# Ocheretovich/tachyon

Measured on AMD Instinct MI355X. Metric: BN254 G1 MSM scalars/s @2^26 and Fr NTT elems/s @2^24, 1/2/4/8 GPU, higher is better.
Workload: dtype u32; 1 GPU; BN254 G1 VariableBaseMSM 2^26 (BASELINE configs[1]), device-resident inputs, result normalised to affine on the host; msm_log_n=26, points_per_gpu=67108864, window_bits=21, windows=12, windows_per_gpu=12, parallelism=msm point shards x1 + RCCL all-gather of partial points, communicator=single GPU

## Files before the change

### include/tachyon_mi355x.h

```cpp
#ifndef TACHYON_MI355X_H_
#define TACHYON_MI355X_H_

#include <stddef.h>
#include <stdint.h>

#define TACHYON_C_EXPORT __attribute__((visibility("default")))

#ifdef __cplusplus
extern "C" {
#endif

typedef struct tachyon_bn254_fq { uint64_t limbs[4]; } tachyon_bn254_fq;
typedef struct tachyon_bn254_fr { uint64_t limbs[4]; } tachyon_bn254_fr;
typedef struct tachyon_bn254_fq2 { tachyon_bn254_fq c0, c1; } tachyon_bn254_fq2;
typedef struct tachyon_bls12_381_fq { uint64_t limbs[6]; } tachyon_bls12_381_fq;
typedef struct tachyon_bls12_381_fr { uint64_t limbs[4]; } tachyon_bls12_381_fr;
typedef struct tachyon_bls12_381_fq2 { tachyon_bls12_381_fq c0, c1; } tachyon_bls12_381_fq2;

#define TACHYON_MI355X_POINT_TYPES(C, G, F)                                   \
  typedef struct tachyon_##C##_##G##_affine { F x, y; } tachyon_##C##_##G##_affine;             \
  typedef struct tachyon_##C##_##G##_point2 { F x, y; } tachyon_##C##_##G##_point2;             \
  typedef struct tachyon_##C##_##G##_jacobian { F x, y, z; } tachyon_##C##_##G##_jacobian;      \
  typedef struct tachyon_##C##_##G##_projective { F x, y, z; } tachyon_##C##_##G##_projective;  \
  typedef struct tachyon_##C##_##G##_xyzz { F x, y, zz, zzz; } tachyon_##C##_##G##_xyzz;
// ... 398 lines not shown
typedef struct tachyon_mi355x_msm_shard {
  size_t start, count;
  unsigned point_groups, window_groups, window_bits, w_begin, w_end;
} tachyon_mi355x_msm_shard;
TACHYON_C_EXPORT int tachyon_mi355x_msm_shard_plan(int curve, size_t n_total, int world, int rank,
                                                  tachyon_mi355x_msm_shard* out);
TACHYON_C_EXPORT int tachyon_mi355x_msm_gpu_sharded_plan_affine(int curve, void* ctx, tachyon_mi355x_comm* comm,
                                                                const tachyon_mi355x_msm_shard* plan,
                                                                const void* bases, const void* scalars,
                                                                void* out_affine);
TACHYON_C_EXPORT int tachyon_mi355x_msm_gpu_run_points(int curve, void* ctx, const void* bases, size_t bases_size,
                                                      int base_form, const void* scalars, size_t scalars_size,
                                                      int form, void* out);
TACHYON_C_EXPORT void tachyon_mi355x_msm_gpu_set_window_bits(int curve, void* ctx, unsigned c);
TACHYON_C_EXPORT int tachyon_mi355x_msm_gpu_set_mixed_windows(int curve, void* ctx, unsigned windows);
TACHYON_C_EXPORT int tachyon_mi355x_msm_mixed_layout(int curve, unsigned windows, unsigned* c_lo, unsigned* n_wide,
                                                     unsigned* key_bits, unsigned* bit_offsets,
                                                     unsigned* bucket_offsets);
TACHYON_C_EXPORT void tachyon_mi355x_msm_gpu_set_profile(int curve, void* ctx, int on);
TACHYON_C_EXPORT int tachyon_mi355x_msm_gpu_set_variant(int curve, void* ctx, int variant);
TACHYON_C_EXPORT void tachyon_mi355x_msm_gpu_last_timings(int curve, const void* ctx, float* out8);
TACHYON_C_EXPORT size_t tachyon_mi355x_msm_gpu_last_divisions(int curve, const void* ctx);
TACHYON_C_EXPORT size_t tachyon_mi355x_msm_gpu_run_bytes(int curve, const void* ctx, size_t size, size_t batch_count);
TACHYON_C_EXPORT size_t tachyon_mi355x_msm_gpu_held_bytes(int curve, const void* ctx);
TACHYON_C_EXPORT unsigned tachyon_mi355x_msm_gpu_last_schedule(int curve, const void* ctx);
TACHYON_C_EXPORT double tachyon_mi355x_msm_madd_ceiling(int curve, int field_bits);
TACHYON_C_EXPORT int tachyon_mi355x_msm_gpu_set_devices(int curve, void* ctx, const int* device_ids, size_t count);
TACHYON_C_EXPORT size_t tachyon_mi355x_msm_gpu_last_shards(int curve, const void* ctx, float* shard_ms,
                                                           size_t* shard_points, int* shard_devices, size_t cap);
TACHYON_C_EXPORT void tachyon_mi355x_msm_plan(int curve, size_t size, unsigned* c, unsigned* windows);
// ... 215 lines not shown
```

### tachyon_amd/_lib.py

```python
import ctypes
import os

HERE = os.path.dirname(os.path.abspath(__file__))
LIB_PATH = os.environ.get("TACHYON_MI355X_LIB") or os.path.join(HERE, "libtachyon_mi355x.so")

CURVES = {"bn254_g1": 0, "bn254_g2": 1, "bls12_381_g1": 2, "bls12_381_g2": 3}
FIELDS = {"bn254_fq": 0, "bn254_fr": 1, "bls12_381_fq": 2, "bls12_381_fr": 3}
FIELD_BYTES = {"bn254_fq": 32, "bn254_fr": 32, "bls12_381_fq": 48, "bls12_381_fr": 32}
CURVE_INFO = {
    "bn254_g1": (64, "bn254_fr"),
    "bn254_g2": (128, "bn254_fr"),
    "bls12_381_g1": (96, "bls12_381_fr"),
    "bls12_381_g2": (192, "bls12_381_fr"),
}

_lib = None

vp, sz, i32, u8, u64 = ctypes.c_void_p, ctypes.c_size_t, ctypes.c_int, ctypes.c_uint8, ctypes.c_uint64
fp = ctypes.POINTER(ctypes.c_float)
COMM_FN = ctypes.CFUNCTYPE(ctypes.c_int, ctypes.c_void_p, ctypes.c_void_p, ctypes.c_void_p, ctypes.c_size_t)


class MsmShard(ctypes.Structure):
    _fields_ = [("start", ctypes.c_size_t), ("count", ctypes.c_size_t), ("point_groups", ctypes.c_uint),
# ... 95 lines not shown
    ("tachyon_mi355x_ntt4_split_log_r", ctypes.c_uint32, [ctypes.c_uint32, ctypes.c_uint32]),
    ("tachyon_mi355x_bn254_ntt4_stage", None, [vp, i32, i32, vp, vp]),
    ("tachyon_mi355x_bn254_ntt4_synchronize", None, [vp]),
    ("tachyon_mi355x_bn254_ntt4_stream", vp, [vp]),
    ("tachyon_bn254_g2_create_msm_gpu", vp, [u8]),
    ("tachyon_bn254_g2_destroy_msm_gpu", None, [vp]),
    ("tachyon_bn254_g2_affine_msm_gpu", vp, [vp, vp, vp, sz]),
    ("tachyon_bls12_381_g2_create_msm_gpu", vp, [u8]),
    ("tachyon_bls12_381_g2_destroy_msm_gpu", None, [vp]),
    ("tachyon_bls12_381_g2_affine_msm_gpu", vp, [vp, vp, vp, sz]),
    ("tachyon_mi355x_msm_gpu_affine", None, [i32, vp, vp, vp, sz, vp]),
    ("tachyon_mi355x_msm_gpu_window_range_affine", None, [i32, vp, vp, vp, sz, ctypes.c_uint, ctypes.c_uint, vp]),
    ("tachyon_mi355x_msm_gpu_batch_affine", i32, [i32, vp, vp, sz, vp, sz, vp]),
    ("tachyon_mi355x_msm_gpu_plan_windows", ctypes.c_uint, [i32, vp, sz]),
    ("tachyon_mi355x_msm_gpu_set_mixed_windows", i32, [i32, vp, ctypes.c_uint]),
    ("tachyon_mi355x_msm_mixed_layout", i32, [i32, ctypes.c_uint] + [vp] * 5),
    ("tachyon_mi355x_msm_gpu_fold_bases", i32, [i32, vp, vp, sz, ctypes.c_uint, vp]),
    ("tachyon_mi355x_msm_gpu_folded_affine", i32, [i32, vp, vp, vp, sz, ctypes.c_uint, vp]),
    ("tachyon_mi355x_msm_gpu_create", vp, [i32, vp]),
    ("tachyon_mi355x_msm_gpu_destroy", None, [i32, vp]),
    ("tachyon_mi355x_msm_gpu_run", i32, [i32, vp, vp, sz, vp, sz, i32, vp]),
    ("tachyon_mi355x_msm_gpu_run_points", i32, [i32, vp, vp, sz, i32, vp, sz, i32, vp]),
    ("tachyon_mi355x_msm_gpu_set_window_bits", None, [i32, vp, ctypes.c_uint]),
    ("tachyon_mi355x_msm_gpu_set_profile", None, [i32, vp, i32]),
    ("tachyon_mi355x_msm_gpu_set_variant", i32, [i32, vp, i32]),
    ("tachyon_mi355x_msm_gpu_last_divisions", sz, [i32, vp]),
    ("tachyon_mi355x_msm_gpu_run_bytes", sz, [i32, vp, sz, sz]),
    ("tachyon_mi355x_msm_gpu_held_bytes", sz, [i32, vp]),
    ("tachyon_mi355x_msm_gpu_last_schedule", ctypes.c_uint, [i32, vp]),
    ("tachyon_mi355x_msm_madd_ceiling", ctypes.c_double, [i32, i32]),
# ... 194 lines not shown
```

### tachyon_amd/csrc/capi/capi_msm.hip

```cpp
#include "../../../include/tachyon_mi355x.h"

#include <algorithm>
#include <cstdio>
#include <cstdlib>
#include <cstring>
#include <memory>
#include <string>
#include <vector>

#include "../dist/comm.h"
#include "../msm/msm.h"
#include "../msm/msm_multi.h"
#include "capi_guard.h"

using namespace tachyon_amd;

namespace {

template <class Curve>
struct MsmCtx {
  msm::MsmGpu<Curve> impl;
  std::unique_ptr<msm::MsmMultiDevice<Curve>> multi;
  std::string input_dir;
  bool log = false;
// ... 494 lines not shown
}
int tachyon_mi355x_msm_gpu_set_mixed_windows(int curve, void* ctx, unsigned windows) {
  if (!ctx || curve < 0 || curve > 3) return 0;
  const unsigned bits = curve < 2 ? Bn254Fr::Config::kModulusBits : Bls381Fr::Config::kModulusBits;
  if (windows && !msm::MsmPlan::mixed_layout_ok(bits, windows)) return 0;
  GUARD_BEGIN
  CURVE_DISPATCH(curve, {
    auto* m = static_cast<MsmCtx<C>*>(ctx);
    if (windows && m->impl.force_window_bits()) return 0;
    if (windows && window_groups_set(m->impl.variant())) return 0;
    m->set([&](auto& g) { g.set_mixed_windows(windows); });
  })
  GUARD_END
  return 1;
}
int tachyon_mi355x_msm_mixed_layout(int curve, unsigned windows, unsigned* c_lo, unsigned* n_wide, unsigned* key_bits,
                                    unsigned* bit_offsets, unsigned* bucket_offsets) {
  if (curve < 0 || curve > 3) return 0;
  const unsigned bits = curve < 2 ? Bn254Fr::Config::kModulusBits : Bls381Fr::Config::kModulusBits;
  if (!msm::MsmPlan::mixed_layout_ok(bits, windows)) return 0;
  GUARD_BEGIN
  const msm::MsmPlan p = msm::MsmPlan::make_mixed(1, bits, windows);
  if (c_lo) *c_lo = p.c;
  if (n_wide) *n_wide = p.n_wide;
  if (key_bits) *key_bits = msm::kMixedKeyBits;
  for (unsigned w = 0; w <= windows; ++w) {
    if (bit_offsets) bit_offsets[w] = p.bit_offset(w);
    if (bucket_offsets) bucket_offsets[w] = (unsigned)p.bucket_offset(w);
  }
  GUARD_END
// ... 109 lines not shown
```

### tachyon_amd/csrc/msm/msm.h

```cpp
#pragma once
#include <hip/hip_runtime.h>

#include <cstddef>
#include <algorithm>
#include <cstdint>
#include <cstdlib>
#include <stdexcept>
#include <string>
#include <vector>

#include "../common/hip_util.h"
#include "../ec/point.h"

namespace tachyon_amd::msm {

constexpr int kMsmVariantMask = 0x3FFFFBF | (1 << 27);
constexpr int kMsmVariantUniformWindows = 1 << 27;
constexpr unsigned kSchedFusedRecode = 1, kSchedRecodeFedSort = 2, kSchedNarrowStaging = 4, kSchedAcc29 = 8,
                   kSchedLanePair = 16, kSchedAcc28 = 32, kSchedChainsChecked = 64, kSchedEntStaged = 128,
                   kSchedMixedWindows = 256;

constexpr unsigned kMixedKeyBits = 24;
constexpr uint32_t kMixedNoKey = (1u << kMixedKeyBits) - 1;

// ... 172 lines not shown
  static size_t fold_table_bytes(size_t points, unsigned fold) { return (size_t)fold * points * sizeof(Aff); }
  static size_t fold_staging_bytes(size_t points, unsigned fold);
  static constexpr size_t kFoldChunkBytes = size_t(1) << 30;

  static Point combine_windows(const std::vector<Point>& window_sums, unsigned c);
  static Point combine_windows(const std::vector<Point>& window_sums, const MsmPlan& plan);
  static double madd_ceiling(int field_bits);

  void set_force_window_bits(unsigned c) { force_c_ = c; }
  void set_mixed_windows(unsigned W) {
    if (W && !MsmPlan::mixed_layout_ok(Fr::Config::kModulusBits, W))
      (void)MsmPlan::make_mixed(1, Fr::Config::kModulusBits, W);
    mixed_w_ = W;
  }
  unsigned mixed_windows() const { return mixed_w_; }
  void set_variant(int v) {
    if (v < 0 || (v & ~kMsmVariantMask)) throw std::runtime_error("tachyon_mi355x: unknown MSM variant bits");
    variant_ = v;
  }
  void set_profile(bool on) { profile_ = on; }
  unsigned force_window_bits() const { return force_c_; }
  int variant() const { return variant_; }
  bool profile() const { return profile_; }
  const MsmTimings& timings() const { return timings_; }
  hipStream_t stream() const { return stream_; }
  unsigned last_levels() const { return last_levels_; }
  size_t last_divisions() const { return last_divisions_; }
  unsigned last_schedule() const { return last_schedule_; }

 private:
// ... 10 lines not shown
  Buffers carve(const Shape& s);
  uint32_t* recode(const Shape& s, const Buffers& b, const Fr* d_scalars);
  void sort_group(const Shape& s, const Buffers& b, unsigned g, size_t e0, size_t ecount, uint32_t* digit_off);
  void upload_pending_bases(const Aff* d_bases, size_t n);
  void early_chain_tables(const Shape& s, const Buffers& b, size_t e0, size_t ecount);
  AccLaunch acc_launch(bool raw, int ent_mode) const;
  void accumulate(const Shape& s, const Buffers& b, const Aff* d_bases, unsigned g, size_t e0, size_t ecount,
                  size_t tbase);
  ReduceKernels reduce_kernels(bool raw) const;
  void check_early_flags(const Shape& s, const Buffers& b);
  void join_offsets(const Shape& s, const Buffers& b, uint32_t nchains, unsigned K2, unsigned levels, uint32_t* ltab,
                    size_t stride);
  void join(const Shape& s, const Buffers& b, const ReduceKernels& rk);
  void window_sums_two_level(const Shape& s, const Buffers& b, const ReduceKernels& rk, Point* d_windows);
  void window_sums_by_trees(const Shape& s, const Buffers& b, Point* d_windows);
  void window_sums(const Shape& s, const Buffers& b, const ReduceKernels& rk, Point* d_windows);
  void window_sums_by_segments(const Shape& s, const Buffers& b, const ReduceKernels& rk, Point* d_windows);
  Point run_host_pipelined(const void* bases, const void* scalars, size_t n, size_t chunks);
  size_t work_bytes(size_t n, unsigned c, size_t batch = 1) const;
  MsmPlan run_plan(size_t n, unsigned c) const;
  struct AccFields {
    bool tree_reduce, acc29, acc28, pair_acc, pair_limb;
  };
  static AccFields acc_fields(int variant);
  struct SlotBytes {
    size_t slot, lvl_slot;
    bool raw;
  };
  static SlotBytes slot_bytes(const AccFields& f, int variant);
  static bool window_sums_by_scan(const AccFields& f, unsigned buckets);
  static unsigned class_seg(unsigned windows, unsigned buckets);
  static size_t mixed_seg_sums(const AccFields& f, unsigned narrow, unsigned W, unsigned B);
  struct SortKnobs {
    bool fuse_recode, rocprim_hist, wide_stage;
    uint32_t spt;
  };
  static SortKnobs sort_knobs(int variant);
  struct SortShape {
    unsigned key_bits, sort_begin, places;
    uint32_t spt;
    bool narrow, fused, own_sort;
    size_t scatter_lds;
  };
  static SortShape sort_shape(const SortKnobs& k, unsigned c, unsigned Ws, unsigned W, unsigned G, size_t entries,
                              bool mixed = false);
  size_t memory_divisions(size_t n, size_t resident_bytes) const;
  void ensure_group_events(unsigned groups);
  void build_chains(const Shape& s, const Buffers& b);
  hipError_t sort_entries(void* tmp, size_t& bytes, const uint64_t* in, uint64_t* out, size_t count,
                          unsigned begin_bit, unsigned end_bit, hipStream_t s);

  hipStream_t stream_ = nullptr;
  bool own_stream_ = false;
  bool profile_ = false;
  unsigned force_c_ = 0;
  unsigned mixed_w_ = 0;
  int variant_ = 0;
  MsmTimings timings_;
  DeviceBuffer bases_, scalars_, ents_, ents2_, sort_tmp_, scan_tmp_, check_;
  DeviceBuffer start_, end_, cnt_, off_a_, off_b_, part_a_, part_b_, seg_a_, seg_b_, windows_, buckets_;
  enum Mark {
    kMarkStart,
    kMarkUploaded,
    kMarkRecoded,
    kMarkSorted,
    kMarkAccumulated,
    kMarkEnd,
    kMarkChainsRead,
    kMarks
  };
  hipEvent_t ev_[kMarks] = {};
// ... 32 lines not shown
```

### tachyon_amd/csrc/msm/msm_impl.h

```cpp
#pragma once
#include "msm.h"
#include "../field/f29.h"
#include "acc29.h"
#include "acc28.h"
#include "acc_pair.h"
#include "pair28.h"
#include "pair29.h"

#include <rocprim/device/device_radix_sort.hpp>
#include <rocprim/device/device_scan.hpp>

#include <algorithm>
#include <cmath>
#include <condition_variable>
#include <cstdlib>
#include <exception>
#include <mutex>
#include <thread>

namespace tachyon_amd::msm {

namespace detail {
namespace {

// ... 436 lines not shown
      k.rsum_pass1 = &window_rsum_pair_kernel<Curve, Fips>;
      k.rsum_pass2 = &window_rsum_total_pair_kernel<Curve, Fips>;
      k.rsum_fix = &window_rsum_fix_pair_kernel<Curve, Fips>;
    }
  }
  if constexpr (std::is_same_v<Curve, Bls381G1>) {
    if (limb28) {
      seg_reduce = raw ? &seg_reduce_kernel<Curve, Limb28ArithT<true, true>> : &seg_reduce_kernel<Curve, Limb28Arith>;
      k.win_segment = raw ? &window_segment_kernel<Curve, Limb28ArithT<true, false>>
                          : &window_segment_kernel<Curve, Limb28Arith>;
      k.win_reduce = &reduce_uniform_kernel<Curve, Limb28Arith>;
    }
  }
  k.level[0][0] = k.level[0][1] = k.level[1][0] = k.level[1][1] = seg_reduce;
  if constexpr (std::is_same_v<Curve, Bn254G1>) {
    if (f.acc29) {
      k.level[0][0] = k.level[0][1] = k.level[1][0] = k.level[1][1] = &seg_reduce29_kernel<false, false>;
      k.win_segment = raw ? &window_segment29_kernel<true> : &window_segment29_kernel<false>;
      k.win_reduce = &reduce_uniform29_kernel;
    }
    if (raw) {
      k.level[1][1] = &seg_reduce29_kernel<true, true>;
      k.level[1][0] = &seg_reduce29_kernel<true, false>;
      k.level[0][1] = &seg_reduce29_kernel<false, true>;
    }
  }
  if constexpr (kG2) {
    if (pair_limb) {
      k.seg1 = &window_seg1_pair_kernel<Curve, LimbPairArith<LimbPol>>;
      k.seg2 = &window_seg2_pair_kernel<Curve, LimbPairArith<LimbPol>>;
      k.comb = &window_combine_pair_kernel<Curve, LimbPairArith<LimbPol>>;
    } else if (f.pair_acc) {
      k.seg1 = &window_seg1_pair_kernel<Curve, FipsPairArith<Curve>>;
      k.seg2 = &window_seg2_pair_kernel<Curve, FipsPairArith<Curve>>;
      k.comb = &window_combine_pair_kernel<Curve, FipsPairArith<Curve>>;
// ... 179 lines not shown
    hipLaunchKernelGGL(rk.rsum_pass1, dim3(grid_for(lanes * (size_t)W * S)), dim3(kBlock), 0, stream_, b.bucket_sum, W,
                       B, s.seg, rs);
    hipLaunchKernelGGL(rk.rsum_pass2, dim3(grid_for(lanes * (size_t)W * S)), dim3(kBlock), 0, stream_, rs, W, B, s.seg,
                       seg_a);
    hipLaunchKernelGGL(rk.rsum_fix, dim3(grid_for(lanes * (size_t)W * S)), dim3(kBlock), 0, stream_, rs, W, B, s.seg,
                       seg_a);
  } else {
    hipLaunchKernelGGL(rk.win_segment, dim3(grid_for(lanes * (size_t)W * S)), dim3(kBlock), 0, stream_, b.bucket_sum, W,
                       B, s.seg, seg_a);
  }
  TA_HIP(hipGetLastError());
  Point* s_cur = seg_a;
  Point* s_nxt = seg_b;
  constexpr unsigned KW = 2;
  while (S > 1) {
    if constexpr (std::is_same_v<Curve, Bn254G1>) {
      if (acc_.acc29 && S <= kBlock) {
        hipLaunchKernelGGL(window_tree29_kernel, dim3(W), dim3(kBlock), 0, stream_, s_cur, S, d_windows);
        TA_HIP(hipGetLastError());
        break;
      }
    }
    unsigned S_out = (S + KW - 1) / KW;
    Point* dst = (S_out == 1) ? d_windows : s_nxt;
    hipLaunchKernelGGL(rk.win_reduce, dim3(grid_for(lanes * (size_t)W * S_out)), dim3(kBlock), 0, stream_, s_cur, W, S,
                       KW, dst);
    TA_HIP(hipGetLastError());
    std::swap(s_cur, s_nxt);
    S = S_out;
  }
  if (B / s.seg == 1) {
    TA_HIP(hipMemcpyAsync(d_windows, seg_a, W * sizeof(Point), hipMemcpyDeviceToDevice, stream_));
  }
}

template <class Curve>
void MsmGpu<Curve>::window_sums(const Shape& s, const Buffers& b, const ReduceKernels& rk, Point* d_windows) {
  if (s.mixed) {
    const unsigned classes[2][3] = {{0, s.narrow, s.B}, {s.narrow, s.W - s.narrow, 2 * s.B}};
    if (const size_t seg_sums = mixed_seg_sums(acc_, s.narrow, s.W, s.B)) {
      seg_a_.ensure(seg_sums * sizeof(Point));
      seg_b_.ensure(seg_sums * sizeof(Point));
    }
    for (const auto& cl : classes) {
      if (cl[1] == 0) continue;
      Shape sc = s;
      Buffers bc = b;
      sc.mixed = false;
      sc.W = cl[1], sc.B = cl[2];
      sc.seg = class_seg(cl[1], cl[2]);
      sc.seg_tree = MsmPlan::seg_tree_for(cl[1], cl[2]);
      bc.bucket_sum = reinterpret_cast<Point*>(reinterpret_cast<char*>(b.bucket_sum) +
                                               (size_t)cl[0] * s.B * s.sb.slot);
      window_sums(sc, bc, rk, d_windows + cl[0]);
    }
    return;
  }
  if (rk.seg1 && (variant_ & (1 << 23)) && !acc_.tree_reduce) return window_sums_two_level(s, b, rk, d_windows);
  if (acc_.tree_reduce) return window_sums_by_trees(s, b, d_windows);
  if constexpr (std::is_same_v<Curve, Bn254G1>) {
    const bool raw = s.sb.raw;
    if (window_sums_by_scan(acc_, s.B)) {
      auto* scan = raw ? &window_scan29_kernel<true> : &window_scan29_kernel<false>;
      hipLaunchKernelGGL(scan, dim3(s.W), dim3(kBlock), 0, stream_, b.bucket_sum, s.B, d_windows);
      TA_HIP(hipGetLastError());
      return;
    }
    if (acc_.acc29 && (variant_ & (1u << 19)) && s.B / s.seg <= kBlock) {
      auto* segtree = raw ? &window_segtree29_kernel<true> : &window_segtree29_kernel<false>;
      hipLaunchKernelGGL(segtree, dim3(s.W), dim3(kBlock), 0, stream_, b.bucket_sum, s.B, s.seg, d_windows);
      TA_HIP(hipGetLastError());
      return;
    }
  }
  window_sums_by_segments(s, b, rk, d_windows);
}

template <class Curve>
void MsmGpu<Curve>::enqueue(const Aff* d_bases, const Fr* d_scalars, size_t n, const MsmPlan& plan,
                            Point* d_windows) {
  const Shape s = make_shape(n, plan);
  const Buffers b = carve(s);
  const ReduceKernels rk = reduce_kernels(s.sb.raw);
  last_schedule_ = (s.ss.fused ? kSchedFusedRecode : 0u) | (s.ss.own_sort ? kSchedRecodeFedSort : 0u) |
                   (s.ss.fused && s.ss.narrow ? kSchedNarrowStaging : 0u) | (s.mixed ? kSchedMixedWindows : 0u);
  if (profile_) TA_HIP(hipEventRecord(ev_[kMarkUploaded], stream_));
  uint32_t* digit_off = recode(s, b, d_scalars);
  TA_HIP(hipEventRecord(ev_[kMarkRecoded], stream_));
  if (b.sort_stream != stream_) TA_HIP(hipStreamWaitEvent(b.sort_stream, ev_[kMarkRecoded], 0));
// ... 174 lines not shown

template <class Curve>
bool MsmGpu<Curve>::window_sums_by_scan(const AccFields& f, unsigned buckets) {
  return std::is_same_v<Curve, Bn254G1> && f.acc29 && !f.tree_reduce && buckets <= detail::kBlock;
}

template <class Curve>
unsigned MsmGpu<Curve>::class_seg(unsigned windows, unsigned buckets) {
  unsigned seg = MsmPlan::seg_for(windows, buckets);
  if constexpr (std::is_same_v<Curve, Bn254G2> || std::is_same_v<Curve, Bls381G2>)
    seg = std::min(buckets, std::min(128u, seg * 2));
  return seg;
}

template <class Curve>
size_t MsmGpu<Curve>::mixed_seg_sums(const AccFields& f, unsigned narrow, unsigned W, unsigned B) {
  const unsigned classes[2][2] = {{narrow, B}, {W - narrow, 2 * B}};
  size_t sums = 0;
  for (const auto& cl : classes)
    if (cl[0] && !window_sums_by_scan(f, cl[1])) sums = std::max(sums, (size_t)cl[0] * (cl[1] / class_seg(cl[0], cl[1])));
  return sums;
}

template <class Curve>
MsmPlan MsmGpu<Curve>::run_plan(size_t n, unsigned c) const {
  MsmPlan plan = MsmPlan::make(n, Fr::Config::kModulusBits, c, range_begin_, range_end_);
  const bool plain = range_begin_ == 0 && range_end_ == ~0u && batch_ == 1 && fold_ == 1 && c == 0 &&
                     (((variant_ >> 2) & 3) == 0 || ((variant_ >> 2) & 3) == 3);
  const unsigned mixed_w = mixed_w_ ? mixed_w_ : (variant_ & kMsmVariantUniformWindows) ? 0u : default_mixed_windows(n);
  if (mixed_w && plain) plan = MsmPlan::make_mixed(n, Fr::Config::kModulusBits, mixed_w);
// ... 80 lines not shown

template <class Curve>
size_t MsmGpu<Curve>::work_bytes(size_t n, unsigned c, size_t batch) const {
  const MsmPlan p = run_plan(n, c);
  const size_t entries = n * p.active();
  const size_t T = (entries + p.K - 1) / p.K;
  size_t bytes = entries * 16 + entries / 2;
  const unsigned W = (unsigned)(p.active() * batch), G = batch > 1 ? W : std::max(1u, std::min(p.group, W));
  if (!sort_shape(sort_knobs(variant_), p.c, p.active(), W, G, entries, p.mixed).own_sort) bytes += entries * 8;
  const SlotBytes sb = slot_bytes(acc_fields(variant_), variant_);
  const size_t slot = sb.slot;
  bytes += 2 * T * slot + (2 * T / kJoinFanLong + T + 2) * sb.lvl_slot;
  bytes += (T + 2) * 4 * 11;
  bytes += (T + 2) * 4 * 12;
  bytes += batch * p.total_buckets() * slot;
  if (p.mixed)
    bytes += 2 * mixed_seg_sums(acc_fields(variant_), p.narrow(), p.windows, p.buckets) * sizeof(Point);
  else if (!window_sums_by_scan(acc_fields(variant_), p.buckets))
    bytes += 2 * batch * p.active() * (p.buckets / p.seg) * sizeof(Point);
  return bytes + bytes / 10;
}

template <class Curve>
size_t MsmGpu<Curve>::held_bytes() const {
  const DeviceBuffer* bufs[] = {&ents_,  &ents2_, &sort_tmp_, &scan_tmp_, &start_, &end_,
                                &cnt_,   &off_a_, &off_b_, &part_a_, &part_b_,  &seg_a_,    &seg_b_, &buckets_,
                                &hist_, &lofs_};
  size_t s = 0;
  for (const DeviceBuffer* b : bufs) s += b->capacity();
  return s;
}
// ... 313 lines not shown
```

### tachyon_amd/csrc/msm/msm_multi.h

```cpp
#pragma once
#include <chrono>
#include <exception>
#include <memory>
#include <thread>
#include <vector>

#include "msm.h"

namespace tachyon_amd::msm {

template <class Curve>
class MsmMultiDevice {
 public:
  using Point = typename MsmGpu<Curve>::Point;
  using Aff = typename MsmGpu<Curve>::Aff;
  using Fr = typename MsmGpu<Curve>::Fr;

  explicit MsmMultiDevice(const std::vector<int>& devices) {
    if (devices.empty()) throw std::runtime_error("tachyon_mi355x: empty device list");
    int count = 0;
    TA_HIP(hipGetDeviceCount(&count));
    for (int d : devices)
      if (d < 0 || d >= count)
        throw std::runtime_error("tachyon_mi355x: device id " + std::to_string(d) + " out of range (" +
// ... 26 lines not shown
  size_t devices() const { return shards_.size(); }
  const std::vector<int> device_ids() const {
    std::vector<int> ids;
    for (auto& s : shards_) ids.push_back(s->device);
    return ids;
  }
  const std::vector<float>& last_shard_ms() const { return shard_ms_; }
  const std::vector<size_t>& last_shard_points() const { return shard_n_; }

  void set_force_window_bits(unsigned c) {
    for (auto& s : shards_) s->msm->set_force_window_bits(c);
  }
  void set_mixed_windows(unsigned W) {
    for (auto& s : shards_) s->msm->set_mixed_windows(W);
  }
  void set_variant(int v) {
    for (auto& s : shards_) s->msm->set_variant(v);
  }
  void set_profile(bool on) {
    for (auto& s : shards_) s->msm->set_profile(on);
  }
  void copy_settings(const MsmGpu<Curve>& from) {
    set_force_window_bits(from.force_window_bits());
    set_mixed_windows(from.mixed_windows());
    set_variant(from.variant());
    set_profile(from.profile());
  }
  const MsmGpu<Curve>& lead() const {
    size_t best = 0;
    for (size_t k = 1; k < shard_n_.size(); ++k)
      if (shard_n_[k] > shard_n_[best]) best = k;
    return *shards_[best]->msm;
  }
  size_t last_divisions() const {
    size_t d = 0;
    for (auto& s : shards_) d = std::max(d, s->msm->last_divisions());
    return d;
  }

// ... 84 lines not shown
```

### tachyon_amd/csrc/msm/msm_window.h

```cpp
#pragma once

namespace tachyon_amd::msm {
namespace detail {
namespace {

template <class F>
__device__ XYZZ<F> small_mul(const XYZZ<F>& P, uint32_t m) {
  XYZZ<F> r = XYZZ<F>::zero();
  if (m == 0 || P.is_zero()) return r;
  int top = 31 - __builtin_clz(m);
  r = P;
  for (int bit = top - 1; bit >= 0; --bit) {
    r = r.dbl();
    if ((m >> bit) & 1) r = r + P;
  }
  return r;
}
template <class Ar>
__device__ typename Ar::A small_mul_ar(const typename Ar::A& P, uint32_t m) {
  if (m == 0 || Ar::is_zero(P)) return Ar::zero();
  typename Ar::A r = P;
  for (int bit = 30 - __builtin_clz(m); bit >= 0; --bit) {
    r = Ar::dbl(r);
    if ((m >> bit) & 1) r = Ar::add(r, P);
// ... 200 lines not shown
  using Fb = typename Ar::Fb;
  const uint32_t h = threadIdx.x & 1u;
  const uint32_t S_out = (S_in + K2 - 1) / K2;
  const uint32_t t = (blockIdx.x * kBlock + threadIdx.x) >> 1;
  if (t >= W * S_out) return;
  const uint32_t w = t / S_out, q = t - w * S_out;
  const uint32_t e0 = q * K2, e1 = min(S_in, e0 + K2);
  const Fb* src = reinterpret_cast<const Fb*>(in) + (size_t)8 * w * S_in;
  typename Ar::A acc = Ar::load(src, e0, h);
  for (uint32_t e = e0 + 1; e < e1; ++e) acc = Ar::add(acc, Ar::load(src, e, h), h != 0);
  Ar::store(reinterpret_cast<Fb*>(out), t, h, acc);
}

template <bool kRaw>
__global__ __launch_bounds__(kBlock, 2) void window_segment29_kernel(const XYZZ<Bn254Fq>* __restrict__ bucket_sum,
                                                                    unsigned W, unsigned B, unsigned L,
                                                                    XYZZ<Bn254Fq>* __restrict__ out) {
  const uint32_t S = B / L;
  const uint32_t t = blockIdx.x * kBlock + threadIdx.x;
  if (t >= W * S) return;
  const uint32_t w = t / S, j = t - w * S;
  const size_t b0 = (size_t)w * B + (size_t)j * L;
  acc29::Pt R{acc29::Acc{}, true}, acc = R;
  for (int k = (int)L - 1; k >= 0; --k) {
    R = acc29::add(R, kRaw ? acc29::load_raw(bucket_sum, b0 + k) : acc29::load_pt(bucket_sum, b0 + k));
    acc = acc29::add(acc, R);
  }
  acc = acc29::add(acc, acc29::small_mul(R, j * L));
  acc29::store_pt(out, t, acc);
}
__global__ __launch_bounds__(kBlock, 2) void window_tree29_kernel(const XYZZ<Bn254Fq>* __restrict__ in, unsigned S,
                                                                 XYZZ<Bn254Fq>* __restrict__ out) {
  __shared__ acc29::Raw sh[kBlock];
  const uint32_t w = blockIdx.x, j = threadIdx.x;
  acc29::Pt v{acc29::Acc{}, true};
  if (j < S) v = acc29::load_pt(in, (size_t)w * S + j);
  unsigned span = 1;
  while (span < S) span <<= 1;
  for (unsigned half = span >> 1; half >= 1; half >>= 1) {
    if (j >= half && j < 2 * half) acc29::store_raw(sh, j - half, v);
    __syncthreads();
    if (j < half) v = acc29::add(v, acc29::load_raw(sh, j));
    __syncthreads();
  }
  if (j == 0) acc29::store_pt(out, w, v);
}
template <bool kRaw>
__global__ __launch_bounds__(kBlock, 2) void window_segtree29_kernel(const XYZZ<Bn254Fq>* __restrict__ bucket_sum,
                                                                    unsigned B, unsigned L,
                                                                    XYZZ<Bn254Fq>* __restrict__ out) {
  __shared__ acc29::Raw sh[kBlock];
  const uint32_t S = B / L;
  const uint32_t w = blockIdx.x, j = threadIdx.x;
// ... 32 lines not shown
    if (j + d < B) v = acc29::add(v, acc29::load_raw(sh, j + d));
    __syncthreads();
  }
  unsigned span = 1;
  while (span < B) span <<= 1;
  for (unsigned half = span >> 1; half >= 1; half >>= 1) {
    if (j >= half && j < 2 * half) acc29::store_raw(sh, j - half, v);
    __syncthreads();
    if (j < half) v = acc29::add(v, acc29::load_raw(sh, j));
    __syncthreads();
  }
  if (j == 0) acc29::store_pt(out, w, v);
}

__global__ __launch_bounds__(kBlock, 2) void reduce_uniform29_kernel(const XYZZ<Bn254Fq>* __restrict__ in, unsigned W,
                                                                    unsigned S_in, unsigned K2,
                                                                    XYZZ<Bn254Fq>* __restrict__ out) {
  const uint32_t S_out = (S_in + K2 - 1) / K2;
  const uint32_t t = blockIdx.x * kBlock + threadIdx.x;
  if (t >= W * S_out) return;
  const uint32_t w = t / S_out, q = t - w * S_out;
  const uint32_t e0 = q * K2, e1 = min(S_in, e0 + K2);
  const XYZZ<Bn254Fq>* src = in + (size_t)w * S_in;
  acc29::Pt acc = acc29::load_pt(src, e0);
  for (uint32_t e = e0 + 1; e < e1; ++e) acc = acc29::add(acc, acc29::load_pt(src, e));
  acc29::store_pt(out, t, acc);
}

template <class Curve, class Ar = FipsArith<Curve>>
__global__ __launch_bounds__(kBlock, AccWaves<Curve>::value) void reduce_uniform_kernel(const XYZZ<typename Curve::F>* __restrict__ in,
                                                                unsigned W, unsigned S_in, unsigned K2,
                                                                XYZZ<typename Curve::F>* __restrict__ out) {
  uint32_t S_out = (S_in + K2 - 1) / K2;
  uint32_t t = blockIdx.x * kBlock + threadIdx.x;
  if (t >= W * S_out) return;
  uint32_t w = t / S_out, q = t - w * S_out;
  uint32_t e0 = q * K2, e1 = min(S_in, e0 + K2);
  const XYZZ<typename Curve::F>* src = in + (size_t)w * S_in;
// ... 58 lines not shown
```

### tachyon_amd/msm.py

```python
import ctypes

import numpy as np

from ._lib import CURVE_INFO, CURVES, FIELD_BYTES, MsmShard, lib

_CREATE = {
    "bn254_g1": ("tachyon_bn254_g1_create_msm_gpu", "tachyon_bn254_g1_destroy_msm_gpu", "tachyon_bn254_g1_affine_msm_gpu"),
    "bn254_g2": ("tachyon_bn254_g2_create_msm_gpu", "tachyon_bn254_g2_destroy_msm_gpu", "tachyon_bn254_g2_affine_msm_gpu"),
    "bls12_381_g1": ("tachyon_bls12_381_g1_create_msm_gpu", "tachyon_bls12_381_g1_destroy_msm_gpu",
                     "tachyon_bls12_381_g1_affine_msm_gpu"),
    "bls12_381_g2": ("tachyon_bls12_381_g2_create_msm_gpu", "tachyon_bls12_381_g2_destroy_msm_gpu",
                     "tachyon_bls12_381_g2_affine_msm_gpu"),
}


def _ptr(x):
    if isinstance(x, (bytes, bytearray)):
        buf = ctypes.create_string_buffer(bytes(x), max(1, len(x)))
        return ctypes.addressof(buf), len(x), buf
    if isinstance(x, np.ndarray):
        if not x.flags["C_CONTIGUOUS"]:
            x = np.ascontiguousarray(x)
        return x.ctypes.data, x.nbytes, x
    if hasattr(x, "data_ptr"):
# ... 129 lines not shown
        if c:
            self._plain_only("set_window_bits")
        lib().tachyon_mi355x_msm_gpu_set_window_bits(self.curve_id, self._ctx, c)
        self.window_bits = c

    def set_mixed_windows(self, windows: int):
        if windows and self.window_bits:
            raise ValueError(f"mixed-width windows refused: window bits are forced to {self.window_bits}")
        if windows and _window_groups(self.variant):
            raise ValueError(f"mixed-width windows refused: variant {self.variant:#x} sets {_window_groups(self.variant)} "
                             "window(s) per sort group (set_variant bits 2-3)")
        if not lib().tachyon_mi355x_msm_gpu_set_mixed_windows(self.curve_id, self._ctx, windows):
            raise ValueError(f"{windows} mixed-width windows refused (widths of 2 to 26 bits, at most 24 key bits)")
        self.mixed_windows = windows

    def set_profile(self, on: bool):
        lib().tachyon_mi355x_msm_gpu_set_profile(self.curve_id, self._ctx, 1 if on else 0)

    def set_variant(self, variant: int):
        if variant >= 0 and _window_groups(variant):
            self._plain_only(f"variant {variant:#x} ({_window_groups(variant)} window(s) per sort group, bits 2-3)")
        if not lib().tachyon_mi355x_msm_gpu_set_variant(self.curve_id, self._ctx, variant):
            raise ValueError(f"unknown MSM variant bits in {variant:#x}")
        self.variant = variant

    def set_devices(self, device_ids):
        ids = list(device_ids)
        arr = (ctypes.c_int * max(1, len(ids)))(*ids)
        if not lib().tachyon_mi355x_msm_gpu_set_devices(self.curve_id, self._ctx, arr, len(ids)):
            raise ValueError(f"device ids out of range: {ids}")
# ... 78 lines not shown
```

Baseline: 957.2 million scalars/s.

## Route BN254 acc29 window sums through a unified segment/reduce/tree pass

After: 974.7 million scalars/s, median of 6. 1.02x the previous value.

```diff
diff --git a/include/tachyon_mi355x.h b/include/tachyon_mi355x.h
--- a/include/tachyon_mi355x.h
+++ b/include/tachyon_mi355x.h
@@ -436,6 +436,7 @@
                                                       int form, void* out);
 TACHYON_C_EXPORT void tachyon_mi355x_msm_gpu_set_window_bits(int curve, void* ctx, unsigned c);
 TACHYON_C_EXPORT int tachyon_mi355x_msm_gpu_set_mixed_windows(int curve, void* ctx, unsigned windows);
+TACHYON_C_EXPORT int tachyon_mi355x_msm_gpu_set_window_segment(int curve, void* ctx, unsigned length);
 TACHYON_C_EXPORT int tachyon_mi355x_msm_mixed_layout(int curve, unsigned windows, unsigned* c_lo, unsigned* n_wide,
                                                      unsigned* key_bits, unsigned* bit_offsets,
                                                      unsigned* bucket_offsets);
diff --git a/tachyon_amd/_lib.py b/tachyon_amd/_lib.py
--- a/tachyon_amd/_lib.py
+++ b/tachyon_amd/_lib.py
@@ -133,6 +133,7 @@
     ("tachyon_mi355x_msm_gpu_batch_affine", i32, [i32, vp, vp, sz, vp, sz, vp]),
     ("tachyon_mi355x_msm_gpu_plan_windows", ctypes.c_uint, [i32, vp, sz]),
     ("tachyon_mi355x_msm_gpu_set_mixed_windows", i32, [i32, vp, ctypes.c_uint]),
+    ("tachyon_mi355x_msm_gpu_set_window_segment", i32, [i32, vp, ctypes.c_uint]),
     ("tachyon_mi355x_msm_mixed_layout", i32, [i32, ctypes.c_uint] + [vp] * 5),
     ("tachyon_mi355x_msm_gpu_fold_bases", i32, [i32, vp, vp, sz, ctypes.c_uint, vp]),
     ("tachyon_mi355x_msm_gpu_folded_affine", i32, [i32, vp, vp, vp, sz, ctypes.c_uint, vp]),
diff --git a/tachyon_amd/csrc/capi/capi_msm.hip b/tachyon_amd/csrc/capi/capi_msm.hip
--- a/tachyon_amd/csrc/capi/capi_msm.hip
+++ b/tachyon_amd/csrc/capi/capi_msm.hip
@@ -532,6 +532,14 @@
   GUARD_END
   return 1;
 }
+int tachyon_mi355x_msm_gpu_set_window_segment(int curve, void* ctx, unsigned length) {
+  if (!ctx || curve < 0 || curve > 3) return 0;
+  if (length && (length < 2 || length > 256 || (length & (length - 1)))) return 0;
+  GUARD_BEGIN
+  CURVE_DISPATCH(curve, static_cast<MsmCtx<C>*>(ctx)->set([&](auto& m) { m.set_window_segment(length); }))
+  GUARD_END
+  return 1;
+}
 int tachyon_mi355x_msm_mixed_layout(int curve, unsigned windows, unsigned* c_lo, unsigned* n_wide, unsigned* key_bits,
                                     unsigned* bit_offsets, unsigned* bucket_offsets) {
   if (curve < 0 || curve > 3) return 0;
diff --git a/tachyon_amd/csrc/msm/msm.h b/tachyon_amd/csrc/msm/msm.h
--- a/tachyon_amd/csrc/msm/msm.h
+++ b/tachyon_amd/csrc/msm/msm.h
@@ -210,6 +210,12 @@
     mixed_w_ = W;
   }
   unsigned mixed_windows() const { return mixed_w_; }
+  void set_window_segment(unsigned L) {
+    if (L && (L < 2 || L > kSeg29Max || (L & (L - 1))))
+      throw std::runtime_error("tachyon_mi355x: a window segment length is a power of two from 2 to 256");
+    seg_force_ = L;
+  }
+  unsigned window_segment() const { return seg_force_; }
   void set_variant(int v) {
     if (v < 0 || (v & ~kMsmVariantMask)) throw std::runtime_error("tachyon_mi355x: unknown MSM variant bits");
     variant_ = v;
@@ -250,6 +256,7 @@
   void join(const Shape& s, const Buffers& b, const ReduceKernels& rk);
   void window_sums_two_level(const Shape& s, const Buffers& b, const ReduceKernels& rk, Point* d_windows);
   void window_sums_by_trees(const Shape& s, const Buffers& b, Point* d_windows);
+  void window_sums29(const Shape& s, const Buffers& b, Point* d_windows);
   void window_sums(const Shape& s, const Buffers& b, const ReduceKernels& rk, Point* d_windows);
   void window_sums_by_segments(const Shape& s, const Buffers& b, const ReduceKernels& rk, Point* d_windows);
   Point run_host_pipelined(const void* bases, const void* scalars, size_t n, size_t chunks);
@@ -265,6 +272,14 @@
   };
   static SlotBytes slot_bytes(const AccFields& f, int variant);
   static bool window_sums_by_scan(const AccFields& f, unsigned buckets);
+  struct Pass29 {
+    unsigned scan_lo, scan_hi, first, narrow, W, L;
+    size_t sums;
+  };
+  static constexpr unsigned kSeg29Max = 256;
+  static bool sums_by_pass29(const AccFields& f);
+  static size_t resident_threads29(bool raw);
+  Pass29 pass29(unsigned narrow, unsigned W, unsigned B, unsigned seg, bool raw) const;
   static unsigned class_seg(unsigned windows, unsigned buckets);
   static size_t mixed_seg_sums(const AccFields& f, unsigned narrow, unsigned W, unsigned B);
   struct SortKnobs {
@@ -291,6 +306,7 @@
   bool profile_ = false;
   unsigned force_c_ = 0;
   unsigned mixed_w_ = 0;
+  unsigned seg_force_ = 0;
   int variant_ = 0;
   MsmTimings timings_;
   DeviceBuffer bases_, scalars_, ents_, ents2_, sort_tmp_, scan_tmp_, check_;
diff --git a/tachyon_amd/csrc/msm/msm_impl.h b/tachyon_amd/csrc/msm/msm_impl.h
--- a/tachyon_amd/csrc/msm/msm_impl.h
+++ b/tachyon_amd/csrc/msm/msm_impl.h
@@ -474,11 +474,7 @@
   }
   k.level[0][0] = k.level[0][1] = k.level[1][0] = k.level[1][1] = seg_reduce;
   if constexpr (std::is_same_v<Curve, Bn254G1>) {
-    if (f.acc29) {
-      k.level[0][0] = k.level[0][1] = k.level[1][0] = k.level[1][1] = &seg_reduce29_kernel<false, false>;
-      k.win_segment = raw ? &window_segment29_kernel<true> : &window_segment29_kernel<false>;
-      k.win_reduce = &reduce_uniform29_kernel;
-    }
+    if (f.acc29) k.level[0][0] = k.level[0][1] = k.level[1][0] = k.level[1][1] = &seg_reduce29_kernel<false, false>;
     if (raw) {
       k.level[1][1] = &seg_reduce29_kernel<true, true>;
       k.level[1][0] = &seg_reduce29_kernel<true, false>;
@@ -688,13 +684,6 @@
   Point* s_nxt = seg_b;
   constexpr unsigned KW = 2;
   while (S > 1) {
-    if constexpr (std::is_same_v<Curve, Bn254G1>) {
-      if (acc_.acc29 && S <= kBlock) {
-        hipLaunchKernelGGL(window_tree29_kernel, dim3(W), dim3(kBlock), 0, stream_, s_cur, S, d_windows);
-        TA_HIP(hipGetLastError());
-        break;
-      }
-    }
     unsigned S_out = (S + KW - 1) / KW;
     Point* dst = (S_out == 1) ? d_windows : s_nxt;
     hipLaunchKernelGGL(rk.win_reduce, dim3(grid_for(lanes * (size_t)W * S_out)), dim3(kBlock), 0, stream_, s_cur, W, S,
@@ -709,7 +698,60 @@
 }
 
 template <class Curve>
+void MsmGpu<Curve>::window_sums29(const Shape& s, const Buffers& b, Point* d_windows) {
+  if constexpr (std::is_same_v<Curve, Bn254G1>) {
+    const bool raw = s.sb.raw;
+    const Pass29 p = pass29(s.mixed ? s.narrow : s.W, s.W, s.B, s.seg, raw);
+    auto buckets_of = [&](unsigned w) {
+      const unsigned units = w + (s.mixed && w > s.narrow ? w - s.narrow : 0u);
+      return reinterpret_cast<Point*>(reinterpret_cast<char*>(b.bucket_sum) + (size_t)units * s.B * s.sb.slot);
+    };
+    auto* scan = raw ? &window_scan29_kernel<true> : &window_scan29_kernel<false>;
+    if (p.scan_lo) {
+      hipLaunchKernelGGL(scan, dim3(p.scan_lo), dim3(kBlock), 0, stream_, b.bucket_sum, s.B, d_windows);
+      TA_HIP(hipGetLastError());
+    }
+    if (p.scan_hi) {
+      hipLaunchKernelGGL(scan, dim3(p.scan_hi), dim3(kBlock), 0, stream_, buckets_of(p.scan_lo), 2 * s.B,
+                         d_windows + p.scan_lo);
+      TA_HIP(hipGetLastError());
+    }
+    if (p.W == 0) return;
+    Point* out = d_windows + p.first;
+    unsigned S = s.B / p.L;
+    const unsigned wide = p.W - p.narrow;
+    Point* s_cur = static_cast<Point*>(seg_a_.ensure(p.sums * sizeof(Point)));
+    Point* s_nxt = static_cast<Point*>(seg_b_.ensure(p.sums * sizeof(Point)));
+    auto* segment = raw ? &window_segment29_kernel<true> : &window_segment29_kernel<false>;
+    hipLaunchKernelGGL(segment, dim3(grid_for(p.sums)), dim3(kBlock), 0, stream_, buckets_of(p.first), p.W, p.narrow, s.B,
+                       p.L, s_cur);
+    TA_HIP(hipGetLastError());
+    while ((wide ? 2 * S : S) > kBlock) {
+      if (wide && (S & 1)) throw std::runtime_error("tachyon_mi355x: odd segment count under windows of two widths");
+      hipLaunchKernelGGL(reduce_uniform29_kernel, dim3(grid_for((size_t)p.narrow * ((S + 1) / 2) + (size_t)wide * S)),
+                         dim3(kBlock), 0, stream_, s_cur, p.W, p.narrow, S, 2u, s_nxt);
+      TA_HIP(hipGetLastError());
+      std::swap(s_cur, s_nxt);
+      S = (S + 1) / 2;
+    }
+    hipLaunchKernelGGL(window_tree29_kernel, dim3(p.W), dim3(kBlock), 0, stream_, s_cur, p.narrow, S, out);
+    TA_HIP(hipGetLastError());
+  }
+}
+
+template <class Curve>
 void MsmGpu<Curve>::window_sums(const Shape& s, const Buffers& b, const ReduceKernels& rk, Point* d_windows) {
+  if (sums_by_pass29(acc_)) {
+    if (!s.mixed && (variant_ & (1u << 19)) && !window_sums_by_scan(acc_, s.B) && s.B / s.seg <= kBlock) {
+      if constexpr (std::is_same_v<Curve, Bn254G1>) {
+        auto* segtree = s.sb.raw ? &window_segtree29_kernel<true> : &window_segtree29_kernel<false>;
+        hipLaunchKernelGGL(segtree, dim3(s.W), dim3(kBlock), 0, stream_, b.bucket_sum, s.B, s.seg, d_windows);
+        TA_HIP(hipGetLastError());
+      }
+      return;
+    }
+    return window_sums29(s, b, d_windows);
+  }
   if (s.mixed) {
     const unsigned classes[2][3] = {{0, s.narrow, s.B}, {s.narrow, s.W - s.narrow, 2 * s.B}};
     if (const size_t seg_sums = mixed_seg_sums(acc_, s.narrow, s.W, s.B)) {
@@ -732,21 +774,6 @@
   }
   if (rk.seg1 && (variant_ & (1 << 23)) && !acc_.tree_reduce) return window_sums_two_level(s, b, rk, d_windows);
   if (acc_.tree_reduce) return window_sums_by_trees(s, b, d_windows);
-  if constexpr (std::is_same_v<Curve, Bn254G1>) {
-    const bool raw = s.sb.raw;
-    if (window_sums_by_scan(acc_, s.B)) {
-      auto* scan = raw ? &window_scan29_kernel<true> : &window_scan29_kernel<false>;
-      hipLaunchKernelGGL(scan, dim3(s.W), dim3(kBlock), 0, stream_, b.bucket_sum, s.B, d_windows);
-      TA_HIP(hipGetLastError());
-      return;
-    }
-    if (acc_.acc29 && (variant_ & (1u << 19)) && s.B / s.seg <= kBlock) {
-      auto* segtree = raw ? &window_segtree29_kernel<true> : &window_segtree29_kernel<false>;
-      hipLaunchKernelGGL(segtree, dim3(s.W), dim3(kBlock), 0, stream_, b.bucket_sum, s.B, s.seg, d_windows);
-      TA_HIP(hipGetLastError());
-      return;
-    }
-  }
   window_sums_by_segments(s, b, rk, d_windows);
 }
 
@@ -951,6 +978,50 @@
 }
 
 template <class Curve>
+bool MsmGpu<Curve>::sums_by_pass29(const AccFields& f) {
+  return std::is_same_v<Curve, Bn254G1> && f.acc29 && !f.tree_reduce;
+}
+
+template <class Curve>
+size_t MsmGpu<Curve>::resident_threads29(bool raw) {
+  static size_t cached[2] = {0, 0};
+  if constexpr (std::is_same_v<Curve, Bn254G1>) {
+    if (!cached[raw]) {
+      int dev = 0, cus = 0, blocks = 0;
+      TA_HIP(hipGetDevice(&dev));
+      TA_HIP(hipDeviceGetAttribute(&cus, hipDeviceAttributeMultiprocessorCount, dev));
+      auto* segment = raw ? &window_segment29_kernel<true> : &window_segment29_kernel<false>;
+      TA_HIP(hipOccupancyMaxActiveBlocksPerMultiprocessor(&blocks, segment, (int)kBlock, 0));
+      cached[raw] = (size_t)std::max(1, blocks) * std::max(1, cus) * kBlock;
+    }
+  }
+  return cached[raw];
+}
+
+template <class Curve>
+typename MsmGpu<Curve>::Pass29 MsmGpu<Curve>::pass29(unsigned narrow, unsigned W, unsigned B, unsigned seg,
+                                                     bool raw) const {
+  Pass29 p{};
+  p.narrow = narrow, p.W = W;
+  if (B <= kBlock) {
+    p.scan_lo = narrow, p.first = narrow, p.narrow = 0, p.W = W - narrow;
+    if (2 * B <= kBlock) p.scan_hi = p.W, p.first = W, p.W = 0;
+  }
+  if (p.W == 0) return p;
+  const size_t nb = ((size_t)p.narrow + 2 * (size_t)(p.W - p.narrow)) * B;
+  if (p.narrow != W) seg = MsmPlan::seg_for(1, (unsigned)std::min<size_t>(nb, 1u << 31));
+  if (seg_force_) {
+    seg = seg_force_;
+  } else if (seg == 64) {
+    const size_t resident = resident_threads29(raw);
+    while (seg < kSeg29Max && nb / seg > resident) seg *= 2;
+  }
+  p.L = std::min(seg, B);
+  p.sums = nb / p.L;
+  return p;
+}
+
+template <class Curve>
 size_t MsmGpu<Curve>::mixed_seg_sums(const AccFields& f, unsigned narrow, unsigned W, unsigned B) {
   const unsigned classes[2][2] = {{narrow, B}, {W - narrow, 2 * B}};
   size_t sums = 0;
@@ -1061,7 +1132,9 @@
   bytes += (T + 2) * 4 * 11;
   bytes += (T + 2) * 4 * 12;
   bytes += batch * p.total_buckets() * slot;
-  if (p.mixed)
+  if (sums_by_pass29(acc_fields(variant_)))
+    bytes += 2 * pass29(p.mixed ? p.narrow() : W, W, p.buckets, p.seg, sb.raw).sums * sizeof(Point);
+  else if (p.mixed)
     bytes += 2 * mixed_seg_sums(acc_fields(variant_), p.narrow(), p.windows, p.buckets) * sizeof(Point);
   else if (!window_sums_by_scan(acc_fields(variant_), p.buckets))
     bytes += 2 * batch * p.active() * (p.buckets / p.seg) * sizeof(Point);
diff --git a/tachyon_amd/csrc/msm/msm_multi.h b/tachyon_amd/csrc/msm/msm_multi.h
--- a/tachyon_amd/csrc/msm/msm_multi.h
+++ b/tachyon_amd/csrc/msm/msm_multi.h
@@ -64,6 +64,9 @@
   void set_mixed_windows(unsigned W) {
     for (auto& s : shards_) s->msm->set_mixed_windows(W);
   }
+  void set_window_segment(unsigned L) {
+    for (auto& s : shards_) s->msm->set_window_segment(L);
+  }
   void set_variant(int v) {
     for (auto& s : shards_) s->msm->set_variant(v);
   }
@@ -73,6 +76,7 @@
   void copy_settings(const MsmGpu<Curve>& from) {
     set_force_window_bits(from.force_window_bits());
     set_mixed_windows(from.mixed_windows());
+    set_window_segment(from.window_segment());
     set_variant(from.variant());
     set_profile(from.profile());
   }
diff --git a/tachyon_amd/csrc/msm/msm_window.h b/tachyon_amd/csrc/msm/msm_window.h
--- a/tachyon_amd/csrc/msm/msm_window.h
+++ b/tachyon_amd/csrc/msm/msm_window.h
@@ -238,29 +238,36 @@
 
 template <bool kRaw>
 __global__ __launch_bounds__(kBlock, 2) void window_segment29_kernel(const XYZZ<Bn254Fq>* __restrict__ bucket_sum,
-                                                                    unsigned W, unsigned B, unsigned L,
+                                                                    unsigned W, unsigned narrow, unsigned B, unsigned L,
                                                                     XYZZ<Bn254Fq>* __restrict__ out) {
   const uint32_t S = B / L;
   const uint32_t t = blockIdx.x * kBlock + threadIdx.x;
-  if (t >= W * S) return;
-  const uint32_t w = t / S, j = t - w * S;
-  const size_t b0 = (size_t)w * B + (size_t)j * L;
+  const uint32_t lo = narrow * S;
+  if (t >= lo + (W - narrow) * 2 * S) return;
+  const uint32_t j = t < lo ? t % S : (t - lo) % (2 * S);
+  const size_t b0 = (size_t)t * L;
+  auto load = [&](size_t i) { return kRaw ? acc29::load_raw(bucket_sum, i) : acc29::load_pt(bucket_sum, i); };
   acc29::Pt R{acc29::Acc{}, true}, acc = R;
-  for (int k = (int)L - 1; k >= 0; --k) {
-    R = acc29::add(R, kRaw ? acc29::load_raw(bucket_sum, b0 + k) : acc29::load_pt(bucket_sum, b0 + k));
+  acc29::Pt next = load(b0 + L - 1);
+  for (int k = (int)L - 1; k >= 0; --k) {
+    const acc29::Pt cur = next;
+    if (k > 0) next = load(b0 + k - 1);
+    R = acc29::add(R, cur);
     acc = acc29::add(acc, R);
   }
   acc = acc29::add(acc, acc29::small_mul(R, j * L));
   acc29::store_pt(out, t, acc);
 }
-__global__ __launch_bounds__(kBlock, 2) void window_tree29_kernel(const XYZZ<Bn254Fq>* __restrict__ in, unsigned S,
-                                                                 XYZZ<Bn254Fq>* __restrict__ out) {
+__global__ __launch_bounds__(kBlock, 2) void window_tree29_kernel(const XYZZ<Bn254Fq>* __restrict__ in, unsigned narrow,
+                                                                 unsigned S, XYZZ<Bn254Fq>* __restrict__ out) {
   __shared__ acc29::Raw sh[kBlock];
   const uint32_t w = blockIdx.x, j = threadIdx.x;
+  const uint32_t Sw = w < narrow ? S : 2 * S;
+  const size_t first = w < narrow ? (size_t)w * S : (size_t)narrow * S + (size_t)(w - narrow) * 2 * S;
   acc29::Pt v{acc29::Acc{}, true};
-  if (j < S) v = acc29::load_pt(in, (size_t)w * S + j);
+  if (j < Sw) v = acc29::load_pt(in, first + j);
   unsigned span = 1;
-  while (span < S) span <<= 1;
+  while (span < Sw) span <<= 1;
   for (unsigned half = span >> 1; half >= 1; half >>= 1) {
     if (j >= half && j < 2 * half) acc29::store_raw(sh, j - half, v);
     __syncthreads();
@@ -323,14 +330,23 @@
 }
 
 __global__ __launch_bounds__(kBlock, 2) void reduce_uniform29_kernel(const XYZZ<Bn254Fq>* __restrict__ in, unsigned W,
-                                                                    unsigned S_in, unsigned K2,
+                                                                    unsigned narrow, unsigned S_in, unsigned K2,
                                                                     XYZZ<Bn254Fq>* __restrict__ out) {
-  const uint32_t S_out = (S_in + K2 - 1) / K2;
+  const uint32_t out_lo = (S_in + K2 - 1) / K2, out_hi = (2 * S_in + K2 - 1) / K2;
   const uint32_t t = blockIdx.x * kBlock + threadIdx.x;
-  if (t >= W * S_out) return;
-  const uint32_t w = t / S_out, q = t - w * S_out;
-  const uint32_t e0 = q * K2, e1 = min(S_in, e0 + K2);
-  const XYZZ<Bn254Fq>* src = in + (size_t)w * S_in;
+  const uint32_t lo = narrow * out_lo;
+  if (t >= lo + (W - narrow) * out_hi) return;
+  uint32_t q, S;
+  size_t first;
+  if (t < lo) {
+    const uint32_t w = t / out_lo;
+    q = t - w * out_lo, S = S_in, first = (size_t)w * S_in;
+  } else {
+    const uint32_t w = (t - lo) / out_hi;
+    q = (t - lo) - w * out_hi, S = 2 * S_in, first = (size_t)narrow * S_in + (size_t)w * 2 * S_in;
+  }
+  const uint32_t e0 = q * K2, e1 = min(S, e0 + K2);
+  const XYZZ<Bn254Fq>* src = in + first;
   acc29::Pt acc = acc29::load_pt(src, e0);
   for (uint32_t e = e0 + 1; e < e1; ++e) acc = acc29::add(acc, acc29::load_pt(src, e));
   acc29::store_pt(out, t, acc);
diff --git a/tachyon_amd/msm.py b/tachyon_amd/msm.py
--- a/tachyon_amd/msm.py
+++ b/tachyon_amd/msm.py
@@ -167,6 +167,10 @@
             raise ValueError(f"{windows} mixed-width windows refused (widths of 2 to 26 bits, at most 24 key bits)")
         self.mixed_windows = windows
 
+    def set_window_segment(self, length: int):
+        if not lib().tachyon_mi355x_msm_gpu_set_window_segment(self.curve_id, self._ctx, length):
+            raise ValueError(f"window segment length {length} refused (a power of two from 2 to 256, or 0)")
+
     def set_profile(self, on: bool):
         lib().tachyon_mi355x_msm_gpu_set_profile(self.curve_id, self._ctx, 1 if on else 0)
 
```
